# nabeelre/BTSbot

Hardware: AMD Instinct MI355X
Metric: alerts/sec (63×63×3 triplet + 25 meta) train+infer, 1/2/4/8 MI355X (higher is better)
Workload: dtype bf16; 1 GPU; BASELINE.json configs[1]: ConvNeXt-pico multi-modal (mm_ConvNeXt) bf16 inference, batch=1024 synthetic triplets per GPU, inputs resident in HBM, logits+scores out; per_gpu_batch=1024, global_batch=1024, precision=bf16, weights=seeded random, layer-scale ~1, parallelism=1 independent replicas, batch-sharded, no collective, pipeline_depth=3

## Files before the change

### btsbot_amd/csrc/backbone_train.hip

```cpp
#include <string.h>

#include "ctx.h"
#include "stage0.h"
#include "stage2p.h"

namespace {

struct BlkBuf {
  float* xin;
  float* d;
  void* xn;
  void* a;
  void* h;
  void* dyT;
  void* da;
  float* dwpart;
  int dwrows;
  float* fS;
  float* Gb;
  float* Sb;
  float* fpart;
};

constexpr size_t WPART_FLOATS = (size_t)16 << 20;
// ... 47 lines not shown
      const bool keep4c = !sc.mlp_bwd[i];
      b.a = keep4c ? take(prows * 4 * ch * esz) : nullptr;
      b.h = keep4c ? take(prows * 4 * ch * esz) : nullptr;
      b.dyT = take(rows * ch * esz);
      b.da = keep4c ? take((rows + 48) * 4 * ch * esz) : nullptr;
      b.dwrows = sc.dwln && dwln_bwd_supported(STAGE_HW[i], (int)ch) ? dwln_bwd_rows(STAGE_HW[i], (int)ch, B) : 0;
      b.dwpart = b.dwrows ? reinterpret_cast<float*>(take((size_t)b.dwrows * 52 * ch * 4)) : nullptr;
      b.fpart = sc.mlp_bwd[i] ? reinterpret_cast<float*>(take(mlp_bwd_part_floats((int)ch, (int)rows) * 4))
                                      : nullptr;
      b.fS = nullptr;
      b.Gb = b.Sb = nullptr;
      k.blk[i].push_back(b);
    }
    k.dyT_down[i] = i > 0 ? take(rows * ch * esz) : nullptr;
    if (rows * ch > maxrc) maxrc = rows * ch;
    if (sc.mlp_bwd[i] && rows * ch * mlp_bwd_planes((int)ch) > maxplanes) maxplanes = rows * ch * mlp_bwd_planes((int)ch);
    if (4 * ch * ch > maxc4c) maxc4c = 4 * ch * ch;
    if (i > 0 && 4 * ch * c.dims[i - 1] > maxc4c) maxc4c = 4 * ch * c.dims[i - 1];
  }
  k.dyA = reinterpret_cast<float*>(take(maxrc * 4));
  k.dyB = reinterpret_cast<float*>(take((maxplanes > maxrc ? maxplanes : maxrc) * 4));
  k.dC = reinterpret_cast<float*>(take(maxrc * 4));
  k.dyT_stem = take((size_t)B * 225 * c.dims[0] * esz);
  for (int i = 0; i < 4; ++i)
    for (auto& b : k.blk[i])
      if (b.fpart != nullptr) b.fS = reinterpret_cast<float*>(take((size_t)c.dims[i] * 4));
  k.fS0 = nullptr;
  for (int i = 0; i < 4 && k.fS0 == nullptr; ++i)
    for (auto& b : k.blk[i])
      if (b.fS != nullptr) {
        k.fS0 = b.fS;
        break;
      }
  k.S = reinterpret_cast<float*>(take((size_t)4 * c.dims[3] * 4));
  k.G = reinterpret_cast<float*>(take(maxc4c * 4));
  k.g_floats = maxc4c;
  k.gb0 = reinterpret_cast<float*>(take(0));
  {
    const size_t start = cur;
    for (int i = 0; i < 4; ++i) {
      const size_t ch = c.dims[i];
      if (!sc.wgrad_batch || sc.mlp_bwd[i] || (ch & 127) != 0 || c.precision == BTSBOT_F32) continue;
      for (auto& b : k.blk[i]) {
        b.Gb = reinterpret_cast<float*>(take(4 * ch * ch * 4));
        b.Sb = reinterpret_cast<float*>(take(ch * 4));
      }
    }
    k.gb_floats = (cur - start) / 4;
  }
  k.dpat = reinterpret_cast<float*>(take(maxpat * 4));
  k.dwpart = reinterpret_cast<float*>(take((size_t)256 * 50 * c.dims[3] * 4));
  k.wpart = reinterpret_cast<float*>(take(2 * WPART_FLOATS * 4));
  k.stem_patches = take((size_t)B * 225 * 48 * esz);
  k.stem_pre = reinterpret_cast<float*>(take((size_t)B * 225 * c.dims[0] * 4));
  k.namax = 2 * (c.depths[0] + c.depths[1] + c.depths[2] + c.depths[3]) + 5;
  k.amax = sc.train_split ? reinterpret_cast<unsigned*>(take((size_t)k.namax * AMAX_WORDS * 4)) : nullptr;
  k.total = cur;
  return k;
}

int train_gemm(const btsbot_ctx* h, int epi, const void* A, size_t w, size_t sw, const float* bias, const float* scale,
               const float* aux, void* out, int M, int N, int K, const unsigned* amax_a, unsigned* amax_out, hipStream_t st) {
  const bool sp = h->sched.train_split;
  const unsigned char* W = h->image(sp ? sw : w);
  if (W == nullptr) {
    btsbot_set_error("training step: the %s filter image of a %d x %d product does not exist on this handle", sp ? "split" : "packed",
                     N, K);
    return BTSBOT_ERR_STATE;
  }
  if (sp)
    return launch_gemm_x2_train(epi, reinterpret_cast<const float*>(A), W, bias, scale, aux, reinterpret_cast<float*>(out), M, N,
                                K, amax_a, amax_out, st);
  return launch_gemm(h->cfg.precision, epi, A, W, bias, scale, aux, out, M, N, K, st);
}

int train_wgrad(const btsbot_ctx* h, const void* D, const void* A, const unsigned* damax, const unsigned* aamax, float* out,
                float* cs, int M, int N, int K, int ldo, hipStream_t st, float* part = nullptr, WgradReduceJob* defer = nullptr) {
  const int prec = h->cfg.precision;
  if (h->sched.train_split)
    return launch_wgrad_x2(reinterpret_cast<const float*>(D), reinterpret_cast<const float*>(A), out, cs, M, N, K, ldo, damax,
                           aamax, st, part, WPART_FLOATS, defer);
  if (defer != nullptr) defer->nsl = 0;
  if (prec != BTSBOT_F32) {
    float* probe = det_alloc(0);
    if (probe != nullptr && cs != nullptr) {
      const int rc = launch_wgrad16(prec, D, A, out, nullptr, M, N, K, ldo, st, part, WPART_FLOATS, defer);
      return rc != BTSBOT_OK ? rc : launch_colsum(prec, D, cs, M, N, st);
    }
    return launch_wgrad16(prec, D, A, out, cs, M, N, K, ldo, st, part, WPART_FLOATS, defer);
  }
  return launch_wgrad_cs_f32(reinterpret_cast<const float*>(D), reinterpret_cast<const float*>(A), out, cs, M, N, K, ldo, st);
}

}

size_t bb_cache_bytes(const btsbot_ctx* h, int B) { return carve_bb(h, nullptr, B).total; }

int backbone_train_forward(btsbot_ctx* h, const float* img, int B, hipStream_t st,
                           float** feat_out) {
  const btsbot_config& c = h->cfg;
  const float* m = h->mirror;
  const Schedule& sc = h->sched;
  BBCache k = carve_bb(h, h->bbcache, B);
  auto stage_in = [&](int i) { return h->blocks[i].empty() ? k.xs[i] : k.blk[i][0].xin; };
  if (sc.s0_keep) {
    TRY(pack_sync_early(h, st));
    Stage0Args a;
    TRY(stage0_args(h, true, &a));
    a.img = img;
    for (int j = 0; j < 2; ++j) {
      a.keep_d[j] = k.blk[0][j].d;
      a.keep_xn[j] = k.blk[0][j].xn;
    }
    a.out = stage_in(1);
    a.keep_stem_pre = k.stem_pre;
    a.tap_stem = k.blk[0][0].xin;
    a.keep_xin1 = k.blk[0][1].xin;
    a.tap_stage = k.xs[0];
    a.keep_patches = k.patches[1];
    a.B = B;
    TRY(launch_stage0b(c.precision, a, st));
  } else if (sc.stem16)
    TRY(launch_stem16(c.precision, img, m + h->stem_w, m + h->stem_b, m + h->stem_lnw, m + h->stem_lnb, stage_in(0), B,
                       c.dims[0], st, k.stem_pre));
  else
    TRY(launch_stem(img, m + h->stem_w, m + h->stem_b, m + h->stem_lnw, m + h->stem_lnb, stage_in(0),
                     B, c.dims[0], st, k.stem_pre));
  TRY(pack_sync(h, st));
  const bool s0t = sc.s0_keep, s1t = sc.s1_keep, s2t = sc.s2_kept(B);
  for (int i = s0t ? 1 : 0; i < 4; ++i) {
    const int ch = c.dims[i], hw = STAGE_HW[i], rows = B * hw * hw;
    if (i > 0 && !(i == 3 && s2t) && !(i == 1 && s0t) && !(i == 2 && s1t)) {
      const int cin = c.dims[i - 1];
      TRY(launch_ln_patch(c.precision, k.xs[i - 1], m + h->down[i].ln_w, m + h->down[i].ln_b,
                           k.patches[i], B, STAGE_HW[i - 1], cin, st));
      TRY(train_gemm(h, EPI_BIAS, k.patches[i], h->down[i].p_w, h->down[i].p_s_w, m + h->down[i].b, nullptr, nullptr,
                      stage_in(i), rows, ch, 4 * cin, nullptr, nullptr, st));
    }
    const size_t nblk = h->blocks[i].size();
    if (i == 1 && s1t) {
      Stage1Args a;
      TRY(stage1_args(h, true, &a));
      a.x_in = stage_in(1);
      for (int j = 0; j < 2; ++j) {
        a.keep_d[j] = k.blk[1][j].d;
        a.keep_xn[j] = k.blk[1][j].xn;
      }
      a.out = stage_in(2);
      a.scratch = k.blk[1][1].xin;
      a.tap_stage = k.xs[1];
      a.keep_patches = k.patches[2];
      a.B = B;
      TRY(launch_stage1b(c.precision, a, st));
      continue;
    }
    if (i == 2 && s2t) {
      Stage2pArgs a;
      TRY(stage2p_args(h, true, &a));
      a.x_in = stage_in(2);
      for (size_t j = 0; j < nblk; ++j) {
        const BlkBuf& sb = k.blk[2][j];
        a.keep[j].xin = j == 0 ? sb.d : sb.xin;
        a.keep[j].xn = sb.xn;
        a.keep[j].a = sb.a;
        a.keep[j].hh = sb.h;
      }
      a.out = stage_in(3);
      a.tap_stage = k.xs[2];
      a.ds_patches = k.patches[3];
      a.B = B;
      a.train = 1;
      a.stamps = h->stamps ? h->stamps + STAMP_S2 : nullptr;
      TRY(launch_stage2p(c.precision, a, st));
      continue;
    }
    for (size_t j = 0; j < nblk; ++j) {
      const BlockPk& b = h->blocks[i][j];
      const BlkBuf& s = k.blk[i][j];
      float* xout = j + 1 < nblk ? k.blk[i][j + 1].xin : k.xs[i];
      TRY(launch_dwconv_ln(c.precision, s.xin, IMG_F32(h, b.p_dw),
                            m + b.dw_b, m + b.ln_w, m + b.ln_b, s.xn, B, hw, ch, st, s.d));
      if (s.fpart != nullptr) {
        TRY(launch_fused_mlp(c.precision, ch, s.xn, IMG(h, b.p_fused), m + b.fc1_b, m + b.fc2_b, m + b.gamma, xout,
                              rows, st, nullptr, nullptr, nullptr, 0, s.xin));
        continue;
      }
      TRY(train_gemm(h, EPI_GELU_SAVE, s.xn, b.p_fc1, b.p_s_fc1, m + b.fc1_b, nullptr, reinterpret_cast<const float*>(s.a), s.h,
                      rows, 4 * ch, ch, nullptr, nullptr, st));
      TRY(train_gemm(h, EPI_RESID, s.h, b.p_fc2, b.p_s_fc2, m + b.fc2_b, m + b.gamma, s.xin, xout, rows, ch, 4 * ch, nullptr,
                      nullptr, st));
    }
  }
  *feat_out = k.xs[3];
  h->bb_saved = true;
  return BTSBOT_OK;
}

int backbone_train_backward(btsbot_ctx* h, const float* img, const float* dfeat, float* grads,
                            int B, hipStream_t st) {
  const btsbot_config& c = h->cfg;
  const float* m = h->mirror;
  const int prec = c.precision;
  const Schedule& sc = h->sched;
  BBCache k = carve_bb(h, h->bbcache, B);
  const bool s2t = sc.s2_kept(B);
  float* dy = k.dyA;
  float* dxn = k.dyB;
  TRY(launch_copy_f32(dy, dfeat, (size_t)B * c.dims[3], st));
  hipStream_t sd = st;
  struct Pend { const float* part; float* dst; int rows, cols; };
  Pend pend[8];
  int npend = 0;
  auto fork = [&]() -> int {
    TRY(side_fork(h, st, &sd));
    for (int q = 0; q < npend; ++q) {
      if (pend[q].cols == 0) TRY(launch_dw3_rows(pend[q].part, pend[q].dst, pend[q].rows, sd));
      else TRY(launch_colsum(BTSBOT_F32, pend[q].part, pend[q].dst, pend[q].rows, pend[q].cols, sd));
    }
    npend = 0;
    return BTSBOT_OK;
  };
  auto join = [&]() -> int {
    if (npend > 0) TRY(fork());
    return side_join(h, st);
  };
  auto add_pend = [&](const float* part, float* dst, int rows, int cols) -> int {
    if (npend == (int)(sizeof(pend) / sizeof(pend[0]))) TRY(fork());
    pend[npend++] = Pend{part, dst, rows, cols};
    return BTSBOT_OK;
  };
  const bool fold_cast = prec != BTSBOT_F32;
  {
    float* z0 = k.fS0 != nullptr ? k.fS0 : k.S;
    TRY(launch_fill0(z0, (size_t)((k.G + k.g_floats) - z0), st));
  }
  const bool sp = sc.train_split;
  if (sp) TRY(launch_fill0(reinterpret_cast<float*>(k.amax), (size_t)k.namax * AMAX_WORDS, st));
  auto amax_rec = [&](int slot) { return k.amax + (size_t)slot * AMAX_WORDS; };
  auto blk_amax = [&](int i, int j) {
    int b = j;
    for (int q = 0; q < i; ++q) b += c.depths[q];
    return 2 * b;
  };
  const bool batching = k.gb_floats > 0 && det_alloc(0) == nullptr;
  if (batching) TRY(launch_fill0(k.gb0, k.gb_floats, st));
  auto next_dyT = [&](int i, int j) -> void* {
    if (j > 0) return k.blk[i][j - 1].dyT;
    return i > 0 ? k.dyT_down[i] : nullptr;
  };
  if (sc.side_stream && h->side != nullptr) sd = h->side;
  TRY(launch_stem_im2col(prec, img, k.stem_patches, B, sd));
  bool dyT_ready = false;
  for (int i = 3; i >= 0; --i) {
    const int ch = c.dims[i], hw = STAGE_HW[i], rows = B * hw * hw, H = 4 * ch;
    WgradBatchJob bj[16];
    int nbj = 0;
    for (int j = (int)h->blocks[i].size() - 1; j >= 0; --j) {
      const BlockPk& b = h->blocks[i][j];
      const BlkBuf& s = k.blk[i][j];
      const float* wdw = IMG_F32(h, b.p_dw);
      const bool batched = batching && s.Gb != nullptr && s.fpart == nullptr && nbj + 2 <= 16;
      unsigned* am_dy = sp ? amax_rec(blk_amax(i, j)) : nullptr;
      unsigned* am_da = sp ? amax_rec(blk_amax(i, j) + 1) : nullptr;
      if (sp)
        TRY(launch_copy_amax(dy, reinterpret_cast<float*>(s.dyT), (long)rows * ch, am_dy, st));
      else if (!dyT_ready)
        TRY(launch_scale_cast(prec, dy, nullptr, s.dyT, (long)rows * ch, ch, st));
      dyT_ready = false;
      WgradReduceJob red[2];
      const bool adjacent = b.dw_b == b.dw_w + 49 * (int64_t)ch && b.ln_w == b.dw_b + ch && b.ln_b == b.ln_w + ch;
      const int planes = s.fpart != nullptr ? mlp_bwd_planes(ch) : 1;
      if (planes > 1 && !(s.dwpart != nullptr && adjacent)) {
        btsbot_set_error("backward: the fused MLP backward of a %d-channel block needs dwln_bwd_kernel behind it", ch);
        return BTSBOT_ERR_STATE;
      }
      const bool dw3 = s.dwpart != nullptr && adjacent && dw3_bwd_active(hw, ch);
      if (i == 2 && s2t && !dw3) {
        btsbot_set_error("backward: stage 2's keeping-form forward kept no depthwise output, but block %d's backward reads it", j);
        return BTSBOT_ERR_STATE;
      }
      if (s.fpart != nullptr) {
        TRY(launch_mlp_bwd(prec, ch, s.xn, s.dyT, IMG(h, b.p_fc1), IMG(h, b.p_fc2t), m + b.fc1_b, dxn, s.fpart,
                            k.G, s.fS, grads + b.fc1_w, grads + b.fc1_b, rows, st, red));
        TRY(fork());
      } else if (sc.s2mlp && b.p_w1tp != 0 && s2mlp_bwd_supported(prec, ch)) {
        TRY(launch_s2mlp_bwd(prec, s.dyT, s.a, IMG(h, b.p_w2tp), IMG(h, b.p_w1tp), s.da, dxn, rows, st));
        if (!batched || sc.fork_per_block) TRY(fork());
      } else {
        TRY(train_gemm(h, EPI_DGELU, s.dyT, b.p_fc2t, b.p_s_fc2t, nullptr, nullptr, reinterpret_cast<const float*>(s.a), s.da,
                        rows, H, ch, am_dy, am_da, st));
        if (!batched || sc.fork_per_block) TRY(fork());
        TRY(train_gemm(h, EPI_PLAIN, s.da, b.p_fc1t, b.p_s_fc1t, nullptr, nullptr, nullptr, dxn, rows, ch, H, am_da, nullptr,
                        st));
      }
      void* nxt = fold_cast ? next_dyT(i, j) : nullptr;
      if (dw3) {
        TRY(launch_dw3ln_bwd(m + b.dw_b, dxn, m + b.ln_w, s.xin, wdw, dy, nxt, prec, s.dwpart, B, st, planes,
                              (size_t)rows * ch));
        TRY(add_pend(s.dwpart, grads + b.dw_w, dw3_rows(B), 0));
      } else if (s.dwpart != nullptr && adjacent) {
        TRY(launch_dwln_bwd(s.d, dxn, m + b.ln_w, s.xin, wdw, dy, nxt, prec, s.dwpart, B, hw, ch, st, planes, (size_t)rows * ch));
        TRY(add_pend(s.dwpart, grads + b.dw_w, dwln_bwd_grid(hw, ch, B), 52 * ch));
      } else if (hw == 1 && sc.dwln && ch <= 640) {
        TRY(launch_ln_dw1_bwd(s.d, dxn, m + b.ln_w, s.xin, wdw, dy, nxt, prec, grads + b.ln_w, grads + b.ln_b,
                               grads + b.dw_w, grads + b.dw_b, rows, ch, st));
      } else {
// ... 81 lines not shown
```

### btsbot_amd/csrc/stage1b.hip

```cpp
#include "stage0.h"
#include "stage_regs.h"
#include <type_traits>

namespace {

constexpr int C = 128, HW = 7, PA = 49, G = 2, NPX = G * PA, CT = 4, HID = 512, KS1 = 8;
constexpr int CN = 256, PO = 9;
constexpr int PITCH = 2 * C + 16;
static_assert(C == StageRegs<CT>::C && PITCH == StageRegs<CT>::PITCH, "ln_regs / regs_to_map derive both from CT");
constexpr int MAPB = NPX * PITCH;
constexpr int CHUNKB = 16384, HALFB = CHUNKB / 2, NCH = HID / 32, NSLOT = 3;
constexpr int PL_ROW = 136 * 8, PL_XQ = 8 * PL_ROW, PL_AL = 2 * PL_XQ, PLB = G * PL_AL;
constexpr int OFF_PL = 2 * CHUNKB;
constexpr int LNP = 4 * C + 16;
template <bool X2> struct S1L {
  static constexpr int PLANES = X2 ? 2 : 1;
  static constexpr int SLB = X2 ? 2 * HALFB : HALFB;
  static constexpr int OFF_W2X = OFF_PL + PLANES * PLB;
  static constexpr int OFF_B1 = OFF_W2X + (X2 ? 2 * SLB : 0);
  static constexpr int OFF_LNW = OFF_B1 + (HID + C) * 4;
  static constexpr int LDS_BYTES = OFF_LNW + 2 * C * 4;
  static_assert(4 * SLB <= PLANES * PLB, "W1 slots + W2 slot 0 inside the planar images");
  static_assert(NPX * LNP <= OFF_PL + PLB && NPX * LNP <= OFF_B1, "the fp32 image lies in ring slots 0, 1 + the planar image");
};
static_assert(MAPB <= 2 * CHUNKB && S1L<false>::LDS_BYTES <= 75264 && S1L<true>::LDS_BYTES <= 160 * 1024, "LDS layout");
constexpr int TW_R = 21, TW_BYTES = TW_R * C * 4 * 4 * 2;
constexpr int PARB = TW_BYTES + 3 * C * 4;
constexpr int PARB_X2 = 2 * TW_BYTES + 3 * C * 4;

#define SC_STAMP(i)                                                                \
  do {                                                                             \
    if (a.stamps != nullptr && blockIdx.x == 0 && threadIdx.x == 0) a.stamps[i] = clock64(); \
    if (a.wgt != nullptr && threadIdx.x == 0 && ((i) == 0 || (i) == 13))           \
      a.wgt[2 * blockIdx.x + ((i) == 13)] = wall_clock64();                        \
  } while (0)

template <typename T, int LOPLANE = 0, bool SAT = false>
__device__ __forceinline__ void regs_to_planar(const f32x16 (&x)[CT], unsigned char* pl, int p, int h) {
  const int al = p >= PA ? 1 : 0, pp = p - al * PA;
  const int y = pp / HW, xx = pp - y * HW;
  unsigned char* dst = pl + al * PL_AL + (xx >> 2) * PL_XQ + y * PL_ROW + (xx & 3) * 2 + h * 32;
#pragma unroll
  for (int ct = 0; ct < CT; ++ct)
#pragma unroll
    for (int r = 0; r < 16; ++r) {
      const T hi = (T)(SAT ? __builtin_amdgcn_fmed3f(x[ct][r], -65504.0f, 65504.0f) : x[ct][r]);
      *reinterpret_cast<T*>(dst + (ct * 32 + 8 * (r >> 2) + (r & 3)) * 8) = hi;
      if (LOPLANE > 0) *reinterpret_cast<T*>(dst + LOPLANE + (ct * 32 + 8 * (r >> 2) + (r & 3)) * 8) = (T)(x[ct][r] - (float)hi);
    }
}

template <typename T, bool X2, int WPS = 2, bool KEEP = false>
__global__ __launch_bounds__(256, WPS) void stage1b_kernel(Stage1Args a) {
  using frag = typename Mfma<T>::frag;
  using DT = typename std::conditional<KEEP, f16_t, T>::type;
  using frag4 = typename Mfma<DT>::frag4;
  extern __shared__ __attribute__((aligned(16))) unsigned char smem[];
  unsigned char* pl = smem + OFF_PL;
  unsigned char* stg = smem;
  using L = S1L<X2>;
  constexpr int SLB = L::SLB;
  constexpr int PLO = X2 ? PLB : 0;
  float* b1s = reinterpret_cast<float*>(smem + L::OFF_B1);
  float* b2s = b1s + HID;
  float* lnws = reinterpret_cast<float*>(smem + L::OFF_LNW);
  float* lnbs = lnws + C;
  auto w1slot = [&](int sl) { return pl + sl * SLB; };
  auto w2slot = [&](int sl) { return sl == 0 ? pl + 3 * SLB : (X2 ? smem + L::OFF_W2X : smem) + (sl - 1) * SLB; };

  const int tid = threadIdx.x, lane = tid & 63, wave = __builtin_amdgcn_readfirstlane(tid >> 6);
  const int lr = lane & 31, h = lane >> 5;
  const bool w1wave = wave < 2;
  const int a0 = blockIdx.x * G;
  const int nal = min(G, a.B - a0);
  const int p = wave * 32 + lr;
  const bool live = p < nal * PA;
  const bool inmap = p < NPX;
  const int pm = inmap ? p : 0;
  const int lnrow = pm * LNP + h * 32;
  SC_STAMP(0);
  auto zero_pads = [&]() {
#pragma unroll
    for (int pn = 0; pn < L::PLANES; ++pn) {
      unsigned char* pb = pl + pn * PLB;
      for (int i = tid; i < 4 * PL_ROW / 16; i += 256) {
        const int blk = i / (PL_ROW / 16), o = i - blk * (PL_ROW / 16);
        *reinterpret_cast<uint4*>(pb + (blk >> 1) * PL_AL + (blk & 1) * PL_XQ + 7 * PL_ROW + o * 16) = make_uint4(0u, 0u, 0u, 0u);
      }
      for (int i = tid; i < G * HW * C; i += 256) {
        const int al = i / (HW * C), r = (i / C) % HW, c = i % C;
        *reinterpret_cast<unsigned short*>(pb + al * PL_AL + PL_XQ + r * PL_ROW + c * 8 + 6) = 0;
      }
    }
  };
  zero_pads();
  const float* xsrc = a.x_in + ((size_t)a0 * PA + (live ? p : 0)) * C;
  float* xscr = a.scratch + ((size_t)a0 * PA + (live ? p : 0)) * C;
  auto load_x = [&](const float* src, f32x16 (&x)[CT]) {
#pragma unroll
    for (int ct = 0; ct < CT; ++ct)
#pragma unroll
      for (int qd = 0; qd < 4; ++qd) {
        const float4 v4 = *reinterpret_cast<const float4*>(src + ct * 32 + 8 * qd + 4 * h);
        x[ct][4 * qd + 0] = live ? v4.x : 0.f;
        x[ct][4 * qd + 1] = live ? v4.y : 0.f;
        x[ct][4 * qd + 2] = live ? v4.z : 0.f;
        x[ct][4 * qd + 3] = live ? v4.w : 0.f;
      }
  };
  {
    f32x16 x0[CT];
    load_x(xsrc, x0);
    if (inmap) regs_to_planar<DT, PLO, KEEP && !std::is_same<T, f16_t>::value>(x0, pl, p, h);
  }
  SC_STAMP(1);

  f32x16 x[CT];
  const int rot = (blockIdx.x * 5 + (blockIdx.x >> 4)) & (NCH - 1);
#pragma unroll
  for (int j = 0; j < 2; ++j) {
    const Stage0Blk& bk = a.blk[j];
    int ln = lane;
    asm volatile("" : "+v"(ln));
    const int dj = ln & 3, db = ln >> 2;
    const float b1v0 = bk.b1[tid], b1v1 = bk.b1[256 + tid];
    const float b2v = bk.gamma[tid & (C - 1)] * bk.b2[tid & (C - 1)];
    const uint2* twsrc = reinterpret_cast<const uint2*>(bk.par) + (2 * wave) * 64 + ln;
    frag4 tw[TW_R], twl[X2 ? TW_R : 1];
#pragma unroll
    for (int r = 0; r < TW_R; ++r) tw[r] = __builtin_bit_cast(frag4, twsrc[r * 512]);
    if (X2) {
#pragma unroll
      for (int r = 0; r < TW_R; ++r) twl[r] = __builtin_bit_cast(frag4, twsrc[TW_BYTES / 8 + r * 512]);
    }
    const float* pf = reinterpret_cast<const float*>(bk.par + (X2 ? 2 : 1) * TW_BYTES);
    float dwbias[2];
#pragma unroll
    for (int gi = 0; gi < 2; ++gi) dwbias[gi] = pf[16 * (2 * wave + gi) + db];
    const float lnv = pf[C + tid];
    SC_STAMP(2 + 5 * j);
    __syncthreads();
    b1s[tid] = b1v0;
    b1s[256 + tid] = b1v1;
    if (tid < C) b2s[tid] = b2v;
    lnws[tid] = lnv;

    const unsigned char* wsrc[4];
    const unsigned char* wsrcl[4];
#pragma unroll
    for (int i = 0; i < 4; ++i) {
      const int pc = wave * 4 + i;
      if (pc < 8) {
        const int m = pc * 4 + (lane >> 4);
        const int hid = (m & ~12) | ((m & 4) << 1) | ((m & 8) >> 1);
        const size_t o = (size_t)hid * (C * 2) + (((lane & 15) ^ (m & 15)) << 4);
        wsrc[i] = bk.w1 + o;
        wsrcl[i] = X2 ? bk.w1_lo + o : nullptr;
      } else {
        const int r = (pc - 8) * 16 + (lane >> 2);
        const size_t o = (size_t)r * (HID * 2) + (((lane & 3) ^ swz4(r)) << 4);
        wsrc[i] = bk.w2g + o;
        wsrcl[i] = X2 ? bk.w2g_lo + o : nullptr;
      }
    }
    const int wstep0 = w1wave ? 32 * C * 2 : 64;
    auto issue = [&](int k) {
      unsigned char* dst = (w1wave ? w1slot(k % NSLOT) : w2slot(k % NSLOT)) + (wave & 1) * 4096;
#pragma unroll
      for (int i = 0; i < 4; ++i)
        __builtin_amdgcn_global_load_lds((gptr_t)(wsrc[i] + (size_t)((k + rot) & (NCH - 1)) * wstep0),
                                         (lptr_t)(dst + i * 1024), 16, 0, 0);
      if (X2) {
#pragma unroll
        for (int i = 0; i < 4; ++i)
          __builtin_amdgcn_global_load_lds((gptr_t)(wsrcl[i] + (size_t)((k + rot) & (NCH - 1)) * wstep0),
                                           (lptr_t)(dst + HALFB + i * 1024), 16, 0, 0);
      }
    };
    auto issue_piece = [&](int k, int i) {
      unsigned char* dst = (w1wave ? w1slot(k % NSLOT) : w2slot(k % NSLOT)) + (wave & 1) * 4096;
      if (X2 && i >= 4)
        __builtin_amdgcn_global_load_lds((gptr_t)(wsrcl[i & 3] + (size_t)((k + rot) & (NCH - 1)) * wstep0),
                                         (lptr_t)(dst + HALFB + (i & 3) * 1024), 16, 0, 0);
      else
        __builtin_amdgcn_global_load_lds((gptr_t)(wsrc[i] + (size_t)((k + rot) & (NCH - 1)) * wstep0),
                                         (lptr_t)(dst + i * 1024), 16, 0, 0);
    };
    SC_STAMP(3 + 5 * j);

    int rofs[11];
#pragma unroll
    for (int sx = 0; sx < 11; ++sx) {
      const int r = sx + dj - 3;
      rofs[sx] = ((unsigned)r < (unsigned)HW ? r : 7) * PL_ROW;
    }
    float v[2][2][16];
#pragma unroll
    for (int gi = 0; gi < 2; ++gi) {
      if (gi == 1) {
#pragma unroll
        for (int r = 0; r < TW_R; ++r) tw[r] = __builtin_bit_cast(frag4, twsrc[r * 512 + 64]);
        if (X2) {
#pragma unroll
          for (int r = 0; r < TW_R; ++r) twl[r] = __builtin_bit_cast(frag4, twsrc[TW_BYTES / 8 + r * 512 + 64]);
        }
      }
      f32x4 acc[G][2][2];
#pragma unroll
      for (int al = 0; al < G; ++al)
#pragma unroll
        for (int yb = 0; yb < 2; ++yb)
#pragma unroll
          for (int xb = 0; xb < 2; ++xb) acc[al][yb][xb] = f32x4{dwbias[gi], dwbias[gi], dwbias[gi], dwbias[gi]};
      const unsigned char* lb = pl + (16 * (2 * wave + gi) + db) * 8;
      frag4 bq[2][G][2], bql[X2 ? 2 : 1][G][X2 ? 2 : 1];
      auto read_step = [&](int sx, int buf) {
#pragma unroll
        for (int al = 0; al < G; ++al)
#pragma unroll
          for (int q = 0; q < 2; ++q) {
            bq[buf][al][q] = __builtin_bit_cast(frag4, *reinterpret_cast<const uint2*>(lb + al * PL_AL + q * PL_XQ + rofs[sx]));
            if (X2)
              bql[buf][al][q] =
                  __builtin_bit_cast(frag4, *reinterpret_cast<const uint2*>(lb + PLB + al * PL_AL + q * PL_XQ + rofs[sx]));
          }
      };
      read_step(0, 0);
#ifdef S1_EXP_NODW
#pragma unroll 1
      for (int sx = 0; sx < 0; ++sx) {
#else
#pragma unroll
      for (int sx = 0; sx < 11; ++sx) {
#endif
#pragma unroll
        for (int al = 0; al < G; ++al)
#pragma unroll
          for (int q = 0; q < 2; ++q) {
            asm volatile("" : "+v"(bq[sx & 1][al][q]));
            if (X2) asm volatile("" : "+v"(bql[X2 ? sx & 1 : 0][al][X2 ? q : 0]));
          }
        if (sx + 1 < 11) read_step(sx + 1, (sx + 1) & 1);
        __builtin_amdgcn_sched_barrier(0);
#pragma unroll
        for (int al = 0; al < G; ++al)
#pragma unroll
          for (int yb = 0; yb < 2; ++yb) {
            const int ky = sx - 4 * yb;
            if (ky < 0 || ky > 6) continue;
#pragma unroll
            for (int rbi = 0; rbi < 3; ++rbi)
#pragma unroll
              for (int xb = 0; xb < 2; ++xb) {
                const int q = xb + rbi - 1;
                if (q < 0 || q > 1) continue;
                if (X2) {
                  acc[al][yb][xb] = Mfma<DT>::m4(twl[ky * 3 + rbi], bq[sx & 1][al][q], acc[al][yb][xb]);
                  acc[al][yb][xb] = Mfma<DT>::m4(tw[ky * 3 + rbi], bql[X2 ? sx & 1 : 0][al][X2 ? q : 0], acc[al][yb][xb]);
                }
                acc[al][yb][xb] = Mfma<DT>::m4(tw[ky * 3 + rbi], bq[sx & 1][al][q], acc[al][yb][xb]);
              }
          }
        __builtin_amdgcn_sched_barrier(0);
      }
#pragma unroll
      for (int al = 0; al < G; ++al)
#pragma unroll
        for (int yb = 0; yb < 2; ++yb)
#pragma unroll
          for (int xb = 0; xb < 2; ++xb)
#pragma unroll
            for (int i = 0; i < 4; ++i) v[gi][al][yb * 8 + xb * 4 + i] = acc[al][yb][xb][i];
    }
    if (KEEP && a.keep_d[j] != nullptr) {
#pragma unroll
      for (int gi = 0; gi < 2; ++gi)
#pragma unroll
        for (int al = 0; al < G; ++al) {
          if (al >= nal) continue;
          float* dst = a.keep_d[j] + (size_t)(a0 + al) * PA * C + 16 * (2 * wave + gi) + db;
#pragma unroll
          for (int yb = 0; yb < 2; ++yb)
#pragma unroll
            for (int xb = 0; xb < 2; ++xb)
              if (yb < 1 || dj < 3) {
#pragma unroll
                for (int i = 0; i < 4; ++i) {
                  if (xb == 1 && i == 3) continue;
                  dst[((4 * yb + dj) * HW + 4 * xb + i) * C] = v[gi][al][yb * 8 + xb * 4 + i];
                }
              }
        }
    }
    SC_STAMP(4 + 5 * j);
    __syncthreads();
    {
      unsigned char* dst = smem + dj * (HW * LNP) + (32 * wave + db) * 4;
#pragma unroll
      for (int gi = 0; gi < 2; ++gi)
#pragma unroll
        for (int al = 0; al < G; ++al)
#pragma unroll
          for (int yb = 0; yb < 2; ++yb)
#pragma unroll
            for (int xb = 0; xb < 2; ++xb)
              if (yb < 1 || dj < 3) {
#pragma unroll
                for (int i = 0; i < 4; ++i) {
                  if (xb == 1 && i == 3) continue;
                  const int col = 4 * xb + i, ofs = (al * PA + 4 * yb * HW + col) * LNP + gi * 64;
                  *reinterpret_cast<float*>(dst + ofs) = v[gi][al][yb * 8 + xb * 4 + i];
                }
              }
    }
    __syncthreads();

    {
      auto lds4 = [](const void* q) { return __builtin_bit_cast(f32x4, *reinterpret_cast<const bf16x8*>(q)); };
      frag xf[KS1], xfl[X2 ? KS1 : 1];
      float xv[64];
#pragma unroll
      for (int ks = 0; ks < KS1; ++ks)
#pragma unroll
        for (int q = 0; q < 2; ++q) {
          const f32x4 r4 = lds4(smem + lnrow + ks * 64 + q * 16);
#pragma unroll
          for (int e = 0; e < 4; ++e) xv[ks * 8 + q * 4 + e] = r4[e];
        }
      asm volatile("s_waitcnt lgkmcnt(0)" ::: "memory");
      __builtin_amdgcn_s_barrier();
      issue(0);
      issue(1);
      if (w1wave) issue(2);
      float s = 0.f;
#pragma unroll
      for (int n = 0; n < 64; ++n) s += xv[n];
      s += __shfl_xor(s, 32, 64);
      const float mean = s * (1.0f / C);
      float q2 = 0.f;
#pragma unroll
      for (int n = 0; n < 64; ++n) {
        xv[n] -= mean;
        q2 += xv[n] * xv[n];
      }
      q2 += __shfl_xor(q2, 32, 64);
      const float rstd = rsqrtf(q2 * (1.0f / C) + LN_EPS);
#pragma unroll
      for (int ks = 0; ks < KS1; ++ks) {
#pragma unroll
        for (int q = 0; q < 2; ++q) {
          const f32x4 w4 = lds4(lnws + ks * 16 + h * 8 + q * 4), b4 = lds4(lnbs + ks * 16 + h * 8 + q * 4);
#pragma unroll
          for (int e = 0; e < 4; ++e) {
            const float y = xv[ks * 8 + q * 4 + e] * rstd * w4[e] + b4[e];
            const T yh = (T)y;
            xf[ks][q * 4 + e] = yh;
            if (X2) xfl[X2 ? ks : 0][q * 4 + e] = (T)(y - (float)yh);
          }
        }
        if (KEEP && live)
          *reinterpret_cast<frag*>(reinterpret_cast<unsigned char*>(a.keep_xn[j]) + ((size_t)a0 * PA + p) * C * 2 + ks * 32 +
                                   h * 16) = xf[ks];
      }
      SC_STAMP(5 + 5 * j);
      float4 xt[4 * CT];
      __builtin_amdgcn_sched_barrier(0);
      {
        const float* src = j == 0 ? xsrc : xscr;
#pragma unroll
        for (int ct = 0; ct < CT; ++ct)
#pragma unroll
          for (int qd = 0; qd < 4; ++qd) xt[4 * ct + qd] = *reinterpret_cast<const float4*>(src + ct * 32 + 8 * qd + 4 * h);
      }
      __builtin_amdgcn_sched_barrier(0);
      auto bias_acc = [&](int k, f32x16& acc) {
        const float* bp = b1s + ((k + rot) & (NCH - 1)) * 32 + 8 * h;
#pragma unroll
        for (int qd = 0; qd < 4; ++qd) {
          const f32x4 bv = __builtin_bit_cast(f32x4, *reinterpret_cast<const bf16x8*>(bp + 4 * (qd & 1) + 16 * (qd >> 1)));
#pragma unroll
          for (int e = 0; e < 4; ++e) acc[4 * qd + e] = bv[e];
        }
      };
      frag a1l[X2 ? KS1 : 1];
      auto read_a1 = [&](int k, frag (&a1)[KS1]) {
        const unsigned char* w1s = w1slot(k % NSLOT);
#pragma unroll
        for (int ks = 0; ks < KS1; ++ks) {
          a1[ks] = *reinterpret_cast<const frag*>(w1s + lr * 256 + (((ks * 2 + h) ^ (lr & 15)) << 4));
          if (X2) a1l[ks] = *reinterpret_cast<const frag*>(w1s + HALFB + lr * 256 + (((ks * 2 + h) ^ (lr & 15)) << 4));
        }
      };
#ifdef S1_LOOPSTAMP
      unsigned long long lts[16];
#define LS(i) do { __builtin_amdgcn_sched_barrier(0); if (ch == 6 || ch == 7) lts[i + 8 * (ch - 6)] = __builtin_amdgcn_s_memtime(); __builtin_amdgcn_sched_barrier(0); } while (0)
#else
#define LS(i)
#endif
      f32x16 hacc[2];
      frag a1[KS1];
      {
        wait_vm<(X2 ? 8 : 4) + 16>();
        asm volatile("s_waitcnt lgkmcnt(0)" ::: "memory");
        __builtin_amdgcn_s_barrier();
        bias_acc(0, hacc[0]);
        read_a1(0, a1);
#pragma unroll
        for (int ks = 0; ks < KS1; ++ks) {
          if (X2) {
            hacc[0] = Mfma<T>::m32(a1l[ks], xf[ks], hacc[0]);
            hacc[0] = Mfma<T>::m32(a1[ks], xfl[ks], hacc[0]);
          }
          hacc[0] = Mfma<T>::m32(a1[ks], xf[ks], hacc[0]);
        }
        __builtin_amdgcn_sched_barrier(0);
        wait_vm<0>();
        asm volatile("s_waitcnt lgkmcnt(0)" ::: "memory");
        __builtin_amdgcn_s_barrier();
        bias_acc(1, hacc[1]);
        read_a1(1, a1);
        __builtin_amdgcn_sched_barrier(0);
#pragma unroll
        for (int ct = 0; ct < CT; ++ct)
#pragma unroll
          for (int qd = 0; qd < 4; ++qd) {
            const f32x4 bv = lds4(b2s + ct * 32 + 8 * qd + 4 * h);
            const float4 v4 = xt[4 * ct + qd];
            x[ct][4 * qd + 0] = (live ? v4.x : 0.f) + bv[0];
            x[ct][4 * qd + 1] = (live ? v4.y : 0.f) + bv[1];
            x[ct][4 * qd + 2] = (live ? v4.z : 0.f) + bv[2];
            x[ct][4 * qd + 3] = (live ? v4.w : 0.f) + bv[3];
          }
#pragma unroll
        for (int ct = 0; ct < CT; ++ct) asm volatile("" : "+v"(x[ct]));
        __builtin_amdgcn_sched_barrier(0);
        if (w1wave) issue(3);
      }
      auto step = [&](auto last_c, int ch, f32x16& hc, f32x16& hn) {
        constexpr bool LAST = decltype(last_c)::value;
        LS(0);
        wait_vm<X2 ? 8 : 4>();
        LS(1);
        asm volatile("s_waitcnt lgkmcnt(0)" ::: "memory");
#ifndef S1_EXP_NOBAR
        __builtin_amdgcn_s_barrier();
#endif
        LS(2);
        frag a2[CT][2], a2l[X2 ? CT : 1][2];
        const unsigned char* w2s = w2slot(ch % NSLOT);
#pragma unroll
        for (int ct = 0; ct < CT; ++ct)
#pragma unroll
          for (int s2 = 0; s2 < 2; ++s2) {
            const int r = ct * 32 + lr;
            a2[ct][s2] = *reinterpret_cast<const frag*>(w2s + r * 64 + (((s2 * 2 + h) ^ swz4(r)) << 4));
            if (X2) a2l[ct][s2] = *reinterpret_cast<const frag*>(w2s + HALFB + r * 64 + (((s2 * 2 + h) ^ swz4(r)) << 4));
          }
        LS(3);
        const int kdma = ch + (w1wave ? 4 : 2);
        __builtin_amdgcn_sched_barrier(0);
        LS(4);
        float g[16];
#pragma unroll
        for (int r = 0; r < 8; ++r) {
          if (!LAST) {
            if (X2) {
              hn = Mfma<T>::m32(a1l[r], xf[r], hn);
              hn = Mfma<T>::m32(a1[r], xfl[r], hn);
            }
            hn = Mfma<T>::m32(a1[r], xf[r], hn);
          }
#ifdef S1_EXP_NOGELU
          g[r] = hc[r];
#else
          g[r] = gelu_for<T>(hc[r]);
#endif
#ifndef S1_EXP_NODMA
          if (X2) issue_piece(kdma, r);
          else if (r & 1) issue_piece(kdma, r >> 1);
#endif
          __builtin_amdgcn_sched_barrier(0);
        }
        LS(5);
        if (!LAST) read_a1(ch + 2, a1);
        frag hf, hfl;
#pragma unroll
        for (int r = 0; r < 8; ++r) {
          hf[r] = (T)g[r];
          if (X2) hfl[r] = (T)(g[r] - (float)hf[r]);
        }
#pragma unroll
        for (int ct = 0; ct < CT; ++ct) {
          if (X2) {
            x[ct] = Mfma<T>::m32(a2l[ct][0], hf, x[ct]);
            x[ct] = Mfma<T>::m32(a2[ct][0], hfl, x[ct]);
          }
          x[ct] = Mfma<T>::m32(a2[ct][0], hf, x[ct]);
#ifdef S1_EXP_NOGELU
          g[8 + 2 * ct] = hc[8 + 2 * ct];
          g[9 + 2 * ct] = hc[9 + 2 * ct];
#else
          g[8 + 2 * ct] = gelu_for<T>(hc[8 + 2 * ct]);
          g[9 + 2 * ct] = gelu_for<T>(hc[9 + 2 * ct]);
#endif
          __builtin_amdgcn_sched_barrier(0);
        }
        if (!LAST) bias_acc(ch + 2, hc);
#pragma unroll
        for (int r = 0; r < 8; ++r) {
          hf[r] = (T)g[8 + r];
          if (X2) hfl[r] = (T)(g[8 + r] - (float)hf[r]);
        }
        LS(6);
#pragma unroll
        for (int ct = 0; ct < CT; ++ct) {
          if (X2) {
            x[ct] = Mfma<T>::m32(a2l[ct][1], hf, x[ct]);
            x[ct] = Mfma<T>::m32(a2[ct][1], hfl, x[ct]);
          }
          x[ct] = Mfma<T>::m32(a2[ct][1], hf, x[ct]);
        }
        LS(7);
      };
#ifndef S1_EXP_NOLOOP
#pragma unroll 1
      for (int ch = 0; ch < NCH - 2; ch += 2) {
        step(std::false_type{}, ch, hacc[0], hacc[1]);
        step(std::false_type{}, ch + 1, hacc[1], hacc[0]);
      }
      step(std::false_type{}, NCH - 2, hacc[0], hacc[1]);
      step(std::true_type{}, NCH - 1, hacc[1], hacc[0]);
#endif
      asm volatile("s_waitcnt lgkmcnt(0)" ::: "memory");
#ifdef S1_LOOPSTAMP
      if (a.wgt != nullptr && blockIdx.x == 0 && tid == 0 && j == 0)
        for (int i = 0; i < 16; ++i) a.wgt[4096 + i] = lts[i];
#endif
      wait_vm<0>();
      if (j == 0) {
        __syncthreads();
        zero_pads();
        if (inmap) regs_to_planar<DT, PLO, KEEP && !std::is_same<T, f16_t>::value>(x, pl, p, h);
        if (live) {
#pragma unroll
          for (int ct = 0; ct < CT; ++ct)
#pragma unroll
            for (int qd = 0; qd < 4; ++qd)
              *reinterpret_cast<float4*>(xscr + ct * 32 + 8 * qd + 4 * h) =
                  make_float4(x[ct][4 * qd], x[ct][4 * qd + 1], x[ct][4 * qd + 2], x[ct][4 * qd + 3]);
        }
      }
    }
    SC_STAMP(6 + 5 * j);
  }
  if (a.tap_stage != nullptr && live) {
    float* tp = a.tap_stage + ((size_t)a0 * PA + p) * C;
#pragma unroll
    for (int ct = 0; ct < CT; ++ct)
#pragma unroll
      for (int qd = 0; qd < 4; ++qd)
        *reinterpret_cast<float4*>(tp + ct * 32 + 8 * qd + 4 * h) =
            make_float4(x[ct][4 * qd], x[ct][4 * qd + 1], x[ct][4 * qd + 2], x[ct][4 * qd + 3]);
  }

  {
    __syncthreads();
    {
      f32x16 xn[CT];
      ln_regs(x, a.ds_lnw, a.ds_lnb, h, xn);
      if (inmap) regs_to_map<T, X2 ? MAPB : 0>(xn, stg, p, h);
    }
    static_assert(2 * MAPB <= L::OFF_B1, "two [pixel][channel] images in front of the bias words");
    constexpr int KSD = 4 * C / 16, RING = X2 ? 8 : 16, NSTEP = 2 * KSD;
    const frag* wsrc = reinterpret_cast<const frag*>(a.ds_w) + lane;
    auto fsrc = [&](int stp) {
      return wsrc + (size_t)((wave + 4 * (stp >> 5)) * KSD + (stp & (KSD - 1))) * (X2 ? 128 : 64);
    };
    frag wq[RING], wql[X2 ? RING : 1];
#pragma unroll
    for (int i = 0; i < RING; ++i) {
      wq[i] = *fsrc(i);
      if (X2) wql[i] = fsrc(i)[64];
    }
    __syncthreads();
    if (KEEP) {
      unsigned char* dst = reinterpret_cast<unsigned char*>(a.keep_patches) + (size_t)a0 * PO * 4 * C * 2;
      for (int i = tid; i < nal * PO * 4 * 16; i += 256) {
        const int c16 = i & 15, q = (i >> 4) & 3, o2 = i >> 6;
        const int g2 = o2 / PO, oo2 = o2 - g2 * PO;
        const int pin2 = g2 * PA + (2 * (oo2 / 3) + (q >> 1)) * HW + 2 * (oo2 % 3) + (q & 1);
        *reinterpret_cast<uint4*>(dst + (size_t)(o2 * 4 + q) * C * 2 + 16 * c16) =
            *reinterpret_cast<const uint4*>(stg + pin2 * PITCH + 16 * c16);
      }
    }
    SC_STAMP(12);
    const int o = lr;
    const bool olive = o < nal * PO;
    const int oc = o < G * PO ? o : 0;
    const int g = oc / PO, oo = oc - g * PO;
    const int oy = oo / 3, ox = oo - oy * 3;
    f32x16 acc;
    constexpr int RPT = KSD / RING;
#ifdef S1_EXP_NODS
#pragma unroll 1
    for (int rd = 0; rd < 0; ++rd) {
#else
#pragma unroll 1
    for (int rd = 0; rd < NSTEP / RING; ++rd) {
#endif
      const int cot = wave + 4 * (rd / RPT);
      if (rd % RPT == 0) {
#pragma unroll
        for (int qd = 0; qd < 4; ++qd) {
          const float4 bv = *reinterpret_cast<const float4*>(a.ds_b + cot * 32 + 8 * qd + 4 * h);
          acc[4 * qd + 0] = bv.x;
          acc[4 * qd + 1] = bv.y;
          acc[4 * qd + 2] = bv.z;
          acc[4 * qd + 3] = bv.w;
        }
      }
#pragma unroll
      for (int i = 0; i < RING; ++i) {
        const int stp = rd * RING + i, ks = stp & (KSD - 1);
        const int q = ks >> 3;
        const int pin = g * PA + (2 * oy + (q >> 1)) * HW + 2 * ox + (q & 1);
        const frag bf = *reinterpret_cast<const frag*>(stg + pin * PITCH + (ks & 7) * 32 + h * 16);
        if (X2) {
          const frag bfl = *reinterpret_cast<const frag*>(stg + MAPB + pin * PITCH + (ks & 7) * 32 + h * 16);
          acc = Mfma<T>::m32(wql[i], bf, acc);
          acc = Mfma<T>::m32(wq[i], bfl, acc);
        }
        acc = Mfma<T>::m32(wq[i], bf, acc);
        if (stp + RING < NSTEP) {
          wq[i] = *fsrc(stp + RING);
          if (X2) wql[i] = fsrc(stp + RING)[64];
        }
      }
      if (rd % RPT == RPT - 1 && olive) {
        float* dst = a.out + ((size_t)a0 * PO + o) * CN + cot * 32 + 4 * h;
#pragma unroll
        for (int qd = 0; qd < 4; ++qd)
          *reinterpret_cast<float4*>(dst + 8 * qd) =
              make_float4(acc[4 * qd], acc[4 * qd + 1], acc[4 * qd + 2], acc[4 * qd + 3]);
      }
    }
    SC_STAMP(13);
  }
}

template <typename T, bool X2>
__global__ void pack_s1par_kernel(const float* __restrict__ taps, const float* __restrict__ dw_b,
                                  const float* __restrict__ ln_w, const float* __restrict__ ln_b,
                                  unsigned char* __restrict__ out) {
  const int idx = blockIdx.x * blockDim.x + threadIdx.x;
  constexpr int NTW = TW_R * C * 16;
  if (idx < NTW) {
    const int k = idx & 3, i = (idx >> 2) & 3, c = (idx >> 4) & (C - 1), r = idx / (16 * C);
    const int ky = r / 3, rb = r % 3 - 1, kx = 4 * rb + k - i + 3;
    const float w = (kx >= 0 && kx < 7) ? taps[(ky * 7 + kx) * C + c] : 0.f;
    const T wh = (T)w;
    reinterpret_cast<T*>(out)[idx] = wh;
    if (X2) reinterpret_cast<T*>(out)[NTW + idx] = (T)(w - (float)wh);
    return;
  }
  const int f = idx - NTW;
  if (f >= 3 * C) return;
  float v;
  if (f < C) v = dw_b[f];
  else if (f < 2 * C) v = ln_w[f - C];
  else v = ln_b[f - 2 * C];
  reinterpret_cast<float*>(out + (X2 ? 2 : 1) * TW_BYTES)[f] = v;
}

template <typename T, bool X2 = false>
__global__ void pack_frag32_kernel(const float* __restrict__ w, T* __restrict__ out, int rows, int cin) {
  const long i = (long)blockIdx.x * blockDim.x + threadIdx.x;
  const int K = 4 * cin;
  if (i >= (long)rows * K) return;
  const int j = (int)(i & 7), l = (int)((i >> 3) & 63);
  const long fs = i >> 9;
  const int ksteps = K / 16;
  const int sk = (int)(fs % ksteps), tile = (int)(fs / ksteps);
  const int row = 32 * tile + (l & 31), k = 16 * sk + 8 * (l >> 5) + j;
  const int q = k / cin, c = k - q * cin;
  const float v = w[((long)row * cin + c) * 4 + q];
  const T vh = (T)v;
  if (X2) {
    out[fs * 1024 + l * 8 + j] = vh;
    out[fs * 1024 + 512 + l * 8 + j] = (T)(v - (float)vh);
  } else {
    out[i] = vh;
  }
}

template <typename T, bool X2 = false, int WPS = 2, bool KEEP = false> int launch_stage1b_t(const Stage1Args& a, hipStream_t st) {
  auto kern = stage1b_kernel<T, X2, WPS, KEEP>;
  static DevOnce attr_set;
  static const int pad = switch_on(SW_S1_ONE_WG) && !X2 ? 90 * 1024 - S1L<X2>::LDS_BYTES : 0;
  const int LDS_BYTES = S1L<X2>::LDS_BYTES + pad;
  if (attr_set.need()) {
    HIP_TRY(hipFuncSetAttribute(reinterpret_cast<const void*>(kern),
                                hipFuncAttributeMaxDynamicSharedMemorySize, (int)LDS_BYTES));
    attr_set.done();
  }
  hipLaunchKernelGGL(kern, dim3((a.B + G - 1) / G), dim3(256), LDS_BYTES, st, a);
  LAUNCH_CHECK();
  return BTSBOT_OK;
}

}

#ifdef STAGE1B_X2_TU
int launch_stage1b_x2(const Stage1Args& a, hipStream_t st) {
  if (a.blk[0].w1_lo == nullptr || a.blk[0].w2g_lo == nullptr || a.blk[1].w1_lo == nullptr || a.blk[1].w2g_lo == nullptr) {
    btsbot_set_error("stage1b: the split mode needs the filters' remainder images (w1_lo, w2g_lo)");
    return BTSBOT_ERR_INVALID_ARG;
  }
  return launch_stage1b_t<f16_t, true, 1>(a, st);
}
int launch_pack_s1par_x2(const float* taps, const float* dw_b, const float* ln_w, const float* ln_b, void* out,
                         hipStream_t st) {
  const dim3 grid((TW_R * C * 16 + 3 * C + 255) / 256), blk(256);
  hipLaunchKernelGGL((pack_s1par_kernel<f16_t, true>), grid, blk, 0, st, taps, dw_b, ln_w, ln_b,
                     reinterpret_cast<unsigned char*>(out));
  LAUNCH_CHECK();
  return BTSBOT_OK;
}
int launch_pack_frag32_x2(const float* src, void* dst, int cout, int cin, hipStream_t st) {
  const long total = (long)cout * 4 * cin;
  hipLaunchKernelGGL((pack_frag32_kernel<f16_t, true>), dim3((unsigned)((total + 255) / 256)), dim3(256), 0, st, src,
                     reinterpret_cast<f16_t*>(dst), cout, cin);
  LAUNCH_CHECK();
  return BTSBOT_OK;
}
#else
int launch_stage1b_x2(const Stage1Args& a, hipStream_t st);
int launch_pack_s1par_x2(const float* taps, const float* dw_b, const float* ln_w, const float* ln_b, void* out,
                         hipStream_t st);
int launch_pack_frag32_x2(const float* src, void* dst, int cout, int cin, hipStream_t st);

size_t s1par_bytes() { return PARB_X2; }

int launch_pack_s1par(int prec, const float* taps, const float* dw_b, const float* ln_w,
                      const float* ln_b, void* out, hipStream_t st) {
  unsigned char* o = reinterpret_cast<unsigned char*>(out);
  const dim3 grid((TW_R * C * 16 + 3 * C + 255) / 256), blk(256);
  if (prec == BTSBOT_BF16)
    hipLaunchKernelGGL((pack_s1par_kernel<bf16_t, false>), grid, blk, 0, st, taps, dw_b, ln_w, ln_b, o);
  else if (prec == BTSBOT_F16)
    hipLaunchKernelGGL((pack_s1par_kernel<f16_t, false>), grid, blk, 0, st, taps, dw_b, ln_w, ln_b, o);
  else if (prec == BTSBOT_F16X2)
    return launch_pack_s1par_x2(taps, dw_b, ln_w, ln_b, out, st);
  else {
    btsbot_set_error("pack_s1par: precision %d is not a 16-bit mode", prec);
    return BTSBOT_ERR_INVALID_ARG;
  }
  LAUNCH_CHECK();
  return BTSBOT_OK;
}

int launch_pack_frag32(int prec, const float* src, void* dst, int cout, int cin, hipStream_t st) {
  const long total = (long)cout * 4 * cin;
  const dim3 grid((unsigned)((total + 255) / 256)), blk(256);
  if (prec == BTSBOT_BF16)
    hipLaunchKernelGGL(pack_frag32_kernel<bf16_t>, grid, blk, 0, st, src, reinterpret_cast<bf16_t*>(dst), cout, cin);
  else if (prec == BTSBOT_F16)
    hipLaunchKernelGGL(pack_frag32_kernel<f16_t>, grid, blk, 0, st, src, reinterpret_cast<f16_t*>(dst), cout, cin);
  else if (prec == BTSBOT_F16X2)
    return launch_pack_frag32_x2(src, dst, cout, cin, st);
  else {
    btsbot_set_error("pack_frag32: precision %d is not a 16-bit mode", prec);
    return BTSBOT_ERR_INVALID_ARG;
  }
  LAUNCH_CHECK();
  return BTSBOT_OK;
}

bool stage1_supported(int prec, int c1, int c2) {
  return (prec == BTSBOT_BF16 || prec == BTSBOT_F16 || prec == BTSBOT_F16X2) && c1 == 128 && c2 == 256;
}

int launch_stage1b(int prec, const Stage1Args& a, hipStream_t st) {
  if (a.B <= 0) return BTSBOT_OK;
  if (a.keep_xn[0] != nullptr) {
    if ((a.keep_d[0] == nullptr) != (a.keep_d[1] == nullptr) || a.keep_xn[1] == nullptr || a.keep_patches == nullptr ||
        a.tap_stage == nullptr || a.scratch == nullptr) {
      btsbot_set_error("stage1b: the training forward needs every kept buffer");
      return BTSBOT_ERR_INVALID_ARG;
    }
    if (prec == BTSBOT_BF16) return launch_stage1b_t<bf16_t, false, 2, true>(a, st);
    if (prec == BTSBOT_F16) return launch_stage1b_t<f16_t, false, 2, true>(a, st);
    btsbot_set_error("stage1b: the training forward runs in the bf16 / f16 modes, not %d", prec);
    return BTSBOT_ERR_INVALID_ARG;
  }
  if (prec == BTSBOT_BF16) return launch_stage1b_t<bf16_t>(a, st);
  if (prec == BTSBOT_F16) return launch_stage1b_t<f16_t>(a, st);
  if (prec == BTSBOT_F16X2) return launch_stage1b_x2(a, st);
  btsbot_set_error("stage1b: unsupported precision %d", prec);
// ... 4 lines not shown
```

Baseline: 3.954 million alerts/s.

## Prefetch stage1b per-block params into LDS and hoist tap loads earlier

Moves the per-block bias, layer-norm and downsample weights into LDS once at kernel start, replacing repeated global loads. The depthwise tap fragments for the second group and the next block are prefetched while the current convolution is still running, rather than loaded just before use. The downsample loop is split so the final round has no conditional prefetch. The trade-off is a larger LDS footprint and more live registers, which could reduce occupancy. A debug-only tap copy is also added.

```diff
diff --git a/btsbot_amd/csrc/backbone_train.hip b/btsbot_amd/csrc/backbone_train.hip
--- a/btsbot_amd/csrc/backbone_train.hip
+++ b/btsbot_amd/csrc/backbone_train.hip
@@ -223,6 +223,8 @@
       a.keep_patches = k.patches[2];
       a.B = B;
       TRY(launch_stage1b(c.precision, a, st));
+      if (h->debug && h->taps[2] != nullptr && B <= h->max_chunk)
+        HIP_TRY(hipMemcpyAsync(h->taps[2], k.xs[1], (size_t)rows * ch * 4, hipMemcpyDeviceToDevice, st));
       continue;
     }
     if (i == 2 && s2t) {
diff --git a/btsbot_amd/csrc/stage1b.hip b/btsbot_amd/csrc/stage1b.hip
--- a/btsbot_amd/csrc/stage1b.hip
+++ b/btsbot_amd/csrc/stage1b.hip
@@ -18,12 +18,13 @@
   static constexpr int SLB = X2 ? 2 * HALFB : HALFB;
   static constexpr int OFF_W2X = OFF_PL + PLANES * PLB;
   static constexpr int OFF_B1 = OFF_W2X + (X2 ? 2 * SLB : 0);
-  static constexpr int OFF_LNW = OFF_B1 + (HID + C) * 4;
-  static constexpr int LDS_BYTES = OFF_LNW + 2 * C * 4;
+  static constexpr int BLKW = HID + 3 * C;
+  static constexpr int OFF_DSW = OFF_B1 + 2 * BLKW * 4;
+  static constexpr int LDS_BYTES = OFF_DSW + (2 * C + CN) * 4;
   static_assert(4 * SLB <= PLANES * PLB, "W1 slots + W2 slot 0 inside the planar images");
   static_assert(NPX * LNP <= OFF_PL + PLB && NPX * LNP <= OFF_B1, "the fp32 image lies in ring slots 0, 1 + the planar image");
 };
-static_assert(MAPB <= 2 * CHUNKB && S1L<false>::LDS_BYTES <= 75264 && S1L<true>::LDS_BYTES <= 160 * 1024, "LDS layout");
+static_assert(MAPB <= 2 * CHUNKB && S1L<false>::LDS_BYTES <= 76800 && S1L<true>::LDS_BYTES <= 144384, "LDS layout");
 constexpr int TW_R = 21, TW_BYTES = TW_R * C * 4 * 4 * 2;
 constexpr int PARB = TW_BYTES + 3 * C * 4;
 constexpr int PARB_X2 = 2 * TW_BYTES + 3 * C * 4;
@@ -61,10 +62,8 @@
   using L = S1L<X2>;
   constexpr int SLB = L::SLB;
   constexpr int PLO = X2 ? PLB : 0;
-  float* b1s = reinterpret_cast<float*>(smem + L::OFF_B1);
-  float* b2s = b1s + HID;
-  float* lnws = reinterpret_cast<float*>(smem + L::OFF_LNW);
-  float* lnbs = lnws + C;
+  float* parw = reinterpret_cast<float*>(smem + L::OFF_B1);
+  float* dsw = reinterpret_cast<float*>(smem + L::OFF_DSW);
   auto w1slot = [&](int sl) { return pl + sl * SLB; };
   auto w2slot = [&](int sl) { return sl == 0 ? pl + 3 * SLB : (X2 ? smem + L::OFF_W2X : smem) + (sl - 1) * SLB; };
 
@@ -93,7 +92,6 @@
       }
     }
   };
-  zero_pads();
   const float* xsrc = a.x_in + ((size_t)a0 * PA + (live ? p : 0)) * C;
   float* xscr = a.scratch + ((size_t)a0 * PA + (live ? p : 0)) * C;
   auto load_x = [&](const float* src, f32x16 (&x)[CT]) {
@@ -108,10 +106,51 @@
         x[ct][4 * qd + 3] = live ? v4.w : 0.f;
       }
   };
+  frag4 tw[TW_R], twl[X2 ? TW_R : 1];
+  float dwbias[2];
+  auto load_taps = [&](int j, int gi, int r0, int r1, int ln) {
+    const uint2* twsrc = reinterpret_cast<const uint2*>(a.blk[j].par) + (2 * wave + gi) * 64 + ln;
+#pragma unroll
+    for (int r = r0; r < r1; ++r) tw[r] = __builtin_bit_cast(frag4, twsrc[r * 512]);
+    if (X2) {
+#pragma unroll
+      for (int r = r0; r < r1; ++r) twl[X2 ? r : 0] = __builtin_bit_cast(frag4, twsrc[TW_BYTES / 8 + r * 512]);
+    }
+  };
+  auto load_dwbias = [&](int j, int ln) {
+    const float* pf = reinterpret_cast<const float*>(a.blk[j].par + (X2 ? 2 : 1) * TW_BYTES);
+#pragma unroll
+    for (int gi = 0; gi < 2; ++gi) dwbias[gi] = pf[16 * (2 * wave + gi) + (ln >> 2)];
+  };
   {
+    float pw[2][4];
+#pragma unroll
+    for (int j = 0; j < 2; ++j) {
+      const Stage0Blk& bk = a.blk[j];
+      pw[j][0] = bk.b1[tid];
+      pw[j][1] = bk.b1[256 + tid];
+      pw[j][2] = bk.gamma[tid & (C - 1)] * bk.b2[tid & (C - 1)];
+      pw[j][3] = reinterpret_cast<const float*>(bk.par + (X2 ? 2 : 1) * TW_BYTES)[C + tid];
+    }
+    const float dsl = *(tid < C ? a.ds_lnw + tid : a.ds_lnb + (tid - C));
+    const float dsb = a.ds_b[tid];
+    load_taps(0, 0, 0, TW_R, lane);
+    load_dwbias(0, lane);
     f32x16 x0[CT];
     load_x(xsrc, x0);
+    __builtin_amdgcn_sched_barrier(0);
+    zero_pads();
     if (inmap) regs_to_planar<DT, PLO, KEEP && !std::is_same<T, f16_t>::value>(x0, pl, p, h);
+#pragma unroll
+    for (int j = 0; j < 2; ++j) {
+      float* bw = parw + j * L::BLKW;
+      bw[tid] = pw[j][0];
+      bw[256 + tid] = pw[j][1];
+      if (tid < C) bw[HID + tid] = pw[j][2];
+      bw[HID + C + tid] = pw[j][3];
+    }
+    dsw[tid] = dsl;
+    dsw[2 * C + tid] = dsb;
   }
   SC_STAMP(1);
 
@@ -123,27 +162,12 @@
     int ln = lane;
     asm volatile("" : "+v"(ln));
     const int dj = ln & 3, db = ln >> 2;
-    const float b1v0 = bk.b1[tid], b1v1 = bk.b1[256 + tid];
-    const float b2v = bk.gamma[tid & (C - 1)] * bk.b2[tid & (C - 1)];
-    const uint2* twsrc = reinterpret_cast<const uint2*>(bk.par) + (2 * wave) * 64 + ln;
-    frag4 tw[TW_R], twl[X2 ? TW_R : 1];
-#pragma unroll
-    for (int r = 0; r < TW_R; ++r) tw[r] = __builtin_bit_cast(frag4, twsrc[r * 512]);
-    if (X2) {
-#pragma unroll
-      for (int r = 0; r < TW_R; ++r) twl[r] = __builtin_bit_cast(frag4, twsrc[TW_BYTES / 8 + r * 512]);
-    }
-    const float* pf = reinterpret_cast<const float*>(bk.par + (X2 ? 2 : 1) * TW_BYTES);
-    float dwbias[2];
-#pragma unroll
-    for (int gi = 0; gi < 2; ++gi) dwbias[gi] = pf[16 * (2 * wave + gi) + db];
-    const float lnv = pf[C + tid];
+    const float* b1s = parw + j * L::BLKW;
+    const float* b2s = b1s + HID;
+    const float* lnws = b2s + C;
+    const float* lnbs = lnws + C;
     SC_STAMP(2 + 5 * j);
     __syncthreads();
-    b1s[tid] = b1v0;
-    b1s[256 + tid] = b1v1;
-    if (tid < C) b2s[tid] = b2v;
-    lnws[tid] = lnv;
 
     const unsigned char* wsrc[4];
     const unsigned char* wsrcl[4];
@@ -197,14 +221,6 @@
     float v[2][2][16];
 #pragma unroll
     for (int gi = 0; gi < 2; ++gi) {
-      if (gi == 1) {
-#pragma unroll
-        for (int r = 0; r < TW_R; ++r) tw[r] = __builtin_bit_cast(frag4, twsrc[r * 512 + 64]);
-        if (X2) {
-#pragma unroll
-          for (int r = 0; r < TW_R; ++r) twl[r] = __builtin_bit_cast(frag4, twsrc[TW_BYTES / 8 + r * 512 + 64]);
-        }
-      }
       f32x4 acc[G][2][2];
 #pragma unroll
       for (int al = 0; al < G; ++al)
@@ -261,6 +277,7 @@
                 acc[al][yb][xb] = Mfma<DT>::m4(tw[ky * 3 + rbi], bq[sx & 1][al][q], acc[al][yb][xb]);
               }
           }
+        if (gi == 0 && sx >= 4) load_taps(j, 1, 3 * (sx - 4), 3 * (sx - 4) + 3, ln);
         __builtin_amdgcn_sched_barrier(0);
       }
 #pragma unroll
@@ -538,6 +555,13 @@
 #endif
       wait_vm<0>();
       if (j == 0) {
+        int l1 = lane;
+        asm volatile("" : "+v"(l1));
+        load_taps(1, 0, 0, TW_R, l1);
+        load_dwbias(1, l1);
+        __builtin_amdgcn_sched_barrier(0);
+      }
+      if (j == 0) {
         __syncthreads();
         zero_pads();
         if (inmap) regs_to_planar<DT, PLO, KEEP && !std::is_same<T, f16_t>::value>(x, pl, p, h);
@@ -567,7 +591,7 @@
     __syncthreads();
     {
       f32x16 xn[CT];
-      ln_regs(x, a.ds_lnw, a.ds_lnb, h, xn);
+      ln_regs(x, dsw, dsw + C, h, xn);
       if (inmap) regs_to_map<T, X2 ? MAPB : 0>(xn, stg, p, h);
     }
     static_assert(2 * MAPB <= L::OFF_B1, "two [pixel][channel] images in front of the bias words");
@@ -600,23 +624,17 @@
     const int g = oc / PO, oo = oc - g * PO;
     const int oy = oo / 3, ox = oo - oy * 3;
     f32x16 acc;
-    constexpr int RPT = KSD / RING;
-#ifdef S1_EXP_NODS
-#pragma unroll 1
-    for (int rd = 0; rd < 0; ++rd) {
-#else
-#pragma unroll 1
-    for (int rd = 0; rd < NSTEP / RING; ++rd) {
-#endif
+    constexpr int RPT = KSD / RING, NRD = NSTEP / RING;
+    auto round = [&](auto last_c, int rd) {
+      constexpr bool LASTRD = decltype(last_c)::value;
       const int cot = wave + 4 * (rd / RPT);
       if (rd % RPT == 0) {
+        const float* bp = dsw + 2 * C + cot * 32 + 4 * h;
 #pragma unroll
         for (int qd = 0; qd < 4; ++qd) {
-          const float4 bv = *reinterpret_cast<const float4*>(a.ds_b + cot * 32 + 8 * qd + 4 * h);
-          acc[4 * qd + 0] = bv.x;
-          acc[4 * qd + 1] = bv.y;
-          acc[4 * qd + 2] = bv.z;
-          acc[4 * qd + 3] = bv.w;
+          const f32x4 bv = __builtin_bit_cast(f32x4, *reinterpret_cast<const bf16x8*>(bp + 8 * qd));
+#pragma unroll
+          for (int e = 0; e < 4; ++e) acc[4 * qd + e] = bv[e];
         }
       }
 #pragma unroll
@@ -627,13 +645,13 @@
         const frag bf = *reinterpret_cast<const frag*>(stg + pin * PITCH + (ks & 7) * 32 + h * 16);
         if (X2) {
           const frag bfl = *reinterpret_cast<const frag*>(stg + MAPB + pin * PITCH + (ks & 7) * 32 + h * 16);
-          acc = Mfma<T>::m32(wql[i], bf, acc);
+          acc = Mfma<T>::m32(wql[X2 ? i : 0], bf, acc);
           acc = Mfma<T>::m32(wq[i], bfl, acc);
         }
         acc = Mfma<T>::m32(wq[i], bf, acc);
-        if (stp + RING < NSTEP) {
+        if (!LASTRD) {
           wq[i] = *fsrc(stp + RING);
-          if (X2) wql[i] = fsrc(stp + RING)[64];
+          if (X2) wql[X2 ? i : 0] = fsrc(stp + RING)[64];
         }
       }
       if (rd % RPT == RPT - 1 && olive) {
@@ -643,7 +661,12 @@
           *reinterpret_cast<float4*>(dst + 8 * qd) =
               make_float4(acc[4 * qd], acc[4 * qd + 1], acc[4 * qd + 2], acc[4 * qd + 3]);
       }
-    }
+    };
+#ifndef S1_EXP_NODS
+#pragma unroll 1
+    for (int rd = 0; rd < NRD - 1; ++rd) round(std::false_type{}, rd);
+    round(std::true_type{}, NRD - 1);
+#endif
     SC_STAMP(13);
   }
 }
```

Measured after the change: 3.992 million alerts/s (median of 6 runs). Within noise of the previous version (+1.0%).
